# impromptuRong/hd_yolo

Measured on NVIDIA B200. Metric: postproc_tiles_per_s, higher is better.
Workload: dtype f32

## Files before the change

hd_yolo_b200/csrc/mask_regions.cu:

```cuda
#include "tma_common.cuh"
#include "mask_common.cuh"

namespace hdy {

constexpr int kRegBoxX = 24, kRegBoxY = 24;
constexpr int kRegNm = 32;
constexpr int kRegThreads = 256;
constexpr int kRegWarps = kRegThreads / 32;
constexpr int kRegList = 512;

template <typename E>
struct RegSmemT {
  E proto[kRegNm][kRegBoxY][kRegBoxX];
  float coef[kRegWarps][kRegNm];
  uint16_t list[kRegList];
  int nlist;
  int pad;
  uint64_t bar;
};
__device__ __forceinline__ float proto_f32(float v) { return v; }
__device__ __forceinline__ float proto_f32(__half v) { return __half2float(v); }

constexpr int kRegCap = 254;
constexpr int kMaxRegionsPerTile = 512;
struct RegionList {
  int32_t count;
  uint16_t det[kRegCap];
};
static_assert(sizeof(RegionList) == 512, "one region list is 512 bytes");
struct PmWorkspace {
  int32_t* large_count;
  int32_t* large_list;
  float* patches;
  RegionList* regions;
  int4* kr;
};
static inline size_t align256(size_t v) { return (v + 255) & ~(size_t)255; }
size_t process_mask_workspace_bytes(long long bs, long long max_det) {
  const long long slots = bs * max_det;
  return 256 + align256((size_t)slots * 4) + align256((size_t)slots * 16) +
         (size_t)slots * kPatchPitch * kPatchPitch * 4 + (size_t)bs * kMaxRegionsPerTile * sizeof(RegionList);
}
static PmWorkspace pm_workspace(void* base, long long slots) {
  PmWorkspace w;
  unsigned char* p = static_cast<unsigned char*>(base);
  w.large_count = reinterpret_cast<int32_t*>(p);
  p += 256;
  w.large_list = reinterpret_cast<int32_t*>(p);
  p += align256((size_t)slots * 4);
  w.kr = reinterpret_cast<int4*>(p);
  p += align256((size_t)slots * 16);
  w.patches = reinterpret_cast<float*>(p);
  p += (size_t)slots * kPatchPitch * kPatchPitch * 4;
  w.regions = reinterpret_cast<RegionList*>(p);
  return w;
}

struct KeptRange {
  float x1d, y1d, x2d, y2d;
  int px0, py0, px1, py1;
};
__device__ __forceinline__ KeptRange kept_range(const float4 b, float rx, float ry, int mw, int mh) {
  KeptRange k;
  k.x1d = __fmul_rn(b.x, rx);
  k.x2d = __fmul_rn(b.z, rx);
  k.y1d = __fmul_rn(b.y, ry);
  k.y2d = __fmul_rn(b.w, ry);
  k.px0 = ceil_to_int_clamped(k.x1d, 0, mw);
  k.px1 = ceil_to_int_clamped(k.x2d, 0, mw);
  k.py0 = ceil_to_int_clamped(k.y1d, 0, mh);
  k.py1 = ceil_to_int_clamped(k.y2d, 0, mh);
  if (!(k.x1d == k.x1d) || !(k.x2d == k.x2d) || !(k.y1d == k.y1d) || !(k.y2d == k.y2d)) k.px1 = k.px0, k.py1 = k.py0;
  return k;
}

__constant__ int c_inv16[17] = {0,     65536, 32768, 21846, 16384, 13108, 10923, 9363, 8192,
                                7282,  6554,  5958,  5462,  5042,  4682,  4370,  4096};

__global__ void __launch_bounds__(256) proto_bin_kernel(const float4* __restrict__ boxes,
                                                        const int32_t* __restrict__ counts, long long n_slots,
                                                        int max_det, int mh, int mw, int rxn, int ryn, float rx,
                                                        float ry, const int32_t* __restrict__ geom4,
                                                        RegionList* __restrict__ regions, int4* __restrict__ kr) {
  const long long slot = (long long)blockIdx.x * blockDim.x + threadIdx.x;
  if (slot >= n_slots) return;
  const int tile = (int)(slot / max_det), d = (int)(slot - (long long)tile * max_det);
  const bool live = d < counts[tile] && !(geom4 && (geom4[4 * slot + 2] <= 0 || geom4[4 * slot + 3] <= 0));
  KeptRange k;
  k.px0 = k.py0 = k.px1 = k.py1 = 0;
  if (live) k = kept_range(boxes[slot], rx, ry, mw, mh);
  kr[slot] = make_int4(k.px0, k.py0, k.px1, k.py1);
  if (k.px1 <= k.px0 || k.py1 <= k.py0) return;
  if (k.px1 - k.px0 > kPatchPitch || k.py1 - k.py0 > kPatchPitch) return;
  const int rx0 = k.px0 / kRegBoxX, rx1 = (k.px1 - 1) / kRegBoxX;
  const int ry0 = k.py0 / kRegBoxY, ry1 = (k.py1 - 1) / kRegBoxY;
  for (int ryy = ry0; ryy <= ry1; ++ryy)
    for (int rxx = rx0; rxx <= rx1; ++rxx) {
      RegionList& R = regions[(size_t)tile * (rxn * ryn) + ryy * rxn + rxx];
      const int pos = atomicAdd(&R.count, 1);
      if (pos < kRegCap) R.det[pos] = (uint16_t)d;
    }
}

template <typename E, typename Emit>
__device__ __forceinline__ void contract_piece(const E (*proto)[kRegBoxY][kRegBoxX], const float* __restrict__ coef_smem,
                                               const int4 kr, int X0, int Y0, int lane, Emit emit) {
  float cf[kRegNm];
#pragma unroll
  for (int c = 0; c < kRegNm; c += 4) {
    const float4 v = *reinterpret_cast<const float4*>(coef_smem + c);
    cf[c] = v.x;
    cf[c + 1] = v.y;
    cf[c + 2] = v.z;
    cf[c + 3] = v.w;
  }
  const int qx0 = max(kr.x, X0), qx1 = min(kr.z, X0 + kRegBoxX);
  const int qy0 = max(kr.y, Y0), qy1 = min(kr.w, Y0 + kRegBoxY);
  const int pw = qx1 - qx0;
  const int inv = c_inv16[pw];
  const int rows_per = (32 * inv) >> 16;
  const int ly = (lane * inv) >> 16, lx = lane - ly * pw;
  if (ly >= rows_per) return;
  const int xx = qx0 + lx, sx = xx - X0;
  for (int yy = qy0 + ly; yy < qy1; yy += rows_per) {
    const int sy = yy - Y0;
    float acc = 0.f;
#pragma unroll
    for (int c = 0; c < kRegNm; ++c) acc = fmaf(cf[c], proto_f32(proto[c][sy][sx]), acc);
    emit(xx - kr.x, yy - kr.y, sigmoidf_ref(acc));
  }
}

struct ListedRide {
  const void* protos;
  const float4* boxes;
  const int64_t* offsets;
  uint32_t* bits;
  int32_t* status;
  const int32_t* list;
  const int32_t* list_count;
  long long capacity_words;
  float rx, ry;
  int nm, mh, mw, ih, iw;
  int ctas;
};
constexpr int kListedTiles = 64;

template <typename E>
__global__ void __launch_bounds__(kRegThreads, 3) proto_patch_kernel(
    const __grid_constant__ CUtensorMap tmap, const float* __restrict__ coef, const int4* __restrict__ krs,
    const int32_t* __restrict__ counts, int max_det, int rxn, int ryn, float* __restrict__ patches,
    const RegionList* __restrict__ regions, const ListedRide LR) {
  extern __shared__ __align__(128) unsigned char smem_raw[];
  if ((int)blockIdx.x < LR.ctas) {
    float* stage = reinterpret_cast<float*>(smem_raw);
    process_mask_body<true, sizeof(E) == 2>(LR.protos, coef, LR.boxes, counts, max_det, LR.nm, LR.mh, LR.mw, LR.ih, LR.iw,
                                            1, LR.rx, LR.ry, nullptr, nullptr, LR.offsets, LR.bits, LR.capacity_words,
                                            LR.status, LR.list, (long long)*LR.list_count,
                                            (long long)(blockIdx.x / kListedTiles), (long long)(LR.ctas / kListedTiles),
                                            (int)(blockIdx.x % kListedTiles), kListedTiles, stage,
                                            stage + kPmStage * kPmStage);
    return;
  }
  const int bid = (int)blockIdx.x - LR.ctas;
  RegSmemT<E>& S = *reinterpret_cast<RegSmemT<E>*>(smem_raw);
  const int t = threadIdx.x, lane = t & 31, warp = t >> 5;
  const int per_tile = rxn * ryn;
  const int tile = bid / per_tile, reg = bid - tile * per_tile;
  const int RY = reg / rxn, RX = reg - RY * rxn;
  const int X0 = RX * kRegBoxX, Y0 = RY * kRegBoxY;
  const RegionList& RL = regions[bid];
  const int listed = RL.count;
  if (listed <= 0) return;
  const bool use_list = listed <= kRegCap;
  const int n = use_list ? listed : min(counts[tile], max_det);

  if (t == 0) {
    mbar_init(&S.bar, 1);
    asm volatile("fence.mbarrier_init.release.cluster;" ::: "memory");
    mbar_arrive_expect_tx(&S.bar, (uint32_t)sizeof(S.proto));
    tma_load_4d(&S.proto[0][0][0], &tmap, X0, Y0, 0, tile, &S.bar);
  }
  bool loaded = false;
  for (int base = 0; base < n; base += kRegList) {
    __syncthreads();
    if (t == 0) S.nlist = 0;
    __syncthreads();
    const int lim = min(base + kRegList, n);
    if (use_list) {
      for (int i = base + t; i < lim; i += kRegThreads) S.list[i - base] = RL.det[i];
      if (t == 0) S.nlist = lim - base;
    } else {
      for (int d = base + t; d < lim; d += kRegThreads) {
        const int4 k = krs[(size_t)tile * max_det + d];
        if (k.z <= k.x || k.w <= k.y) continue;
        if (k.z - k.x > kPatchPitch || k.w - k.y > kPatchPitch) continue;
        if (k.z <= X0 || k.x >= X0 + kRegBoxX || k.w <= Y0 || k.y >= Y0 + kRegBoxY) continue;
        S.list[atomicAdd(&S.nlist, 1)] = (uint16_t)(d - base);
      }
    }
    __syncthreads();
    const int nl = S.nlist;
    int e = warp;
    size_t nslot = 0;
    int4 nkr = make_int4(0, 0, 0, 0);
    float ncoef = 0.f;
    auto fetch = [&](int ee) {
      nslot = (size_t)tile * max_det + (use_list ? 0 : base) + S.list[ee];
      nkr = krs[nslot];
      ncoef = coef[nslot * kRegNm + lane];
    };
    if (e < nl) fetch(e);
    if (!loaded) {
      while (!mbar_try_wait(&S.bar, 0)) {
      }
      loaded = true;
    }
    for (; e < nl; e += kRegWarps) {
      const size_t slot = nslot;
      const int4 k = nkr;
      __syncwarp();
      S.coef[warp][lane] = ncoef;
      __syncwarp();
      if (e + kRegWarps < nl) fetch(e + kRegWarps);
      float* dst = patches + slot * (kPatchPitch * kPatchPitch);
      contract_piece<E>(S.proto, S.coef[warp], k, X0, Y0, lane,
                        [&](int px, int py, float v) { dst[py * kPatchPitch + px] = v; });
    }
  }
  if (!loaded) {
    while (!mbar_try_wait(&S.bar, 0)) {
    }
  }
}

constexpr int kUpWarps = 8;
constexpr int kPatchRing = kPatchPitch + 2;
constexpr int kRowChunk = 64;

struct RowTab {
  int i0, i1;
  float l0, l1;
};

struct UpSmem {
  float patch[kUpWarps][kPatchRing * kPatchRing];
  float col[kUpWarps][kPatchRing][32];
  RowTab rows[kUpWarps][kRowChunk];
};

template <bool PACKED, bool UPSAMPLE>
__global__ void __launch_bounds__(kUpWarps * 32) mask_upsample_pack_kernel(
    const float* __restrict__ patches, const float4* __restrict__ boxes, const int32_t* __restrict__ counts,
    long long n_slots, int max_det, int mh, int mw, int ih, int iw, float rx, float ry, float* __restrict__ out_dense,
    const int32_t* __restrict__ geom4, const int64_t* __restrict__ offsets, uint32_t* __restrict__ bits,
    long long capacity_words,
    int32_t* __restrict__ status, int32_t* __restrict__ large_count, int32_t* __restrict__ large_list) {
  static_assert(!(PACKED && UPSAMPLE), "the packed + upsampled form runs mask_upsample_pack2_kernel");
  __shared__ UpSmem S;
  const int lane = threadIdx.x & 31, warp = threadIdx.x >> 5;
  const long long slot = (long long)blockIdx.x * kUpWarps + warp;
  if (slot >= n_slots) return;
  const int tile = (int)(slot / max_det), d = (int)(slot - (long long)tile * max_det);
  if (d >= counts[tile]) return;
  PMGeom g;
  if (geom4) {
    const KeptRange k = kept_range(boxes[slot], rx, ry, mw, mh);
    const int4 wdw = reinterpret_cast<const int4*>(geom4)[slot];
    g.x1d = k.x1d, g.y1d = k.y1d, g.x2d = k.x2d, g.y2d = k.y2d;
    g.px0 = k.px0, g.py0 = k.py0, g.px1 = k.px1, g.py1 = k.py1;
    g.x0 = wdw.x, g.y0 = wdw.y, g.w = wdw.z, g.h = wdw.w;
  } else {
    g = pm_geometry(boxes[slot], mh, mw, ih, iw, UPSAMPLE ? 1 : 0, rx, ry);
  }
  if (g.w <= 0 || g.h <= 0) return;
  const int wpr = (g.w + 31) >> 5;
  const int oh = UPSAMPLE ? ih : mh, ow = UPSAMPLE ? iw : mw;
  long long off = 0;
  if (PACKED) {
    off = offsets[slot];
    if (off + (long long)wpr * g.h > capacity_words) {
      if (lane == 0) atomicOr(status, HDY_STATUS_OVERFLOW);
      return;
    }
  }
  const int pw = g.px1 - g.px0, ph = g.py1 - g.py0;
  if (pw > kPatchPitch || ph > kPatchPitch) {
    if (PACKED)
      for (long long i = lane; i < (long long)wpr * g.h; i += 32) bits[off + i] = 0u;
    if (lane == 0) large_list[atomicAdd(large_count, 1)] = (int32_t)slot;
    return;
  }
  float* P = S.patch[warp];
  {
    const float* src = patches + slot * (kPatchPitch * kPatchPitch);
#pragma unroll
    for (int i = lane; i < kPatchPitch * kPatchPitch; i += 32) {
      const int y = i >> 4, x = i & 15;
      P[(y + 1) * kPatchRing + x + 1] = (y < ph && x < pw) ? src[i] : 0.f;
    }
    for (int i = lane; i < 4 * kPatchRing; i += 32) {
      const int k = i / kPatchRing, j = i - k * kPatchRing;
      const int idx = k == 0 ? j : (k == 1 ? (kPatchRing - 1) * kPatchRing + j : (k == 2 ? j * kPatchRing : j * kPatchRing + kPatchRing - 1));
      P[idx] = 0.f;
    }
  }
  __syncwarp();

  if (!UPSAMPLE) {
    for (int w = 0; w < wpr; ++w) {
      const int c = (w << 5) + lane;
      const bool valid = c < g.w;
      for (int r = 0; r < g.h; ++r) {
        const bool bit = valid && P[(r + 1) * kPatchRing + (valid ? c + 1 : 0)] > 0.5f;
        if (PACKED) {
          const unsigned word = __ballot_sync(0xffffffffu, bit);
          if (lane == 0) bits[off + (long long)r * wpr + w] = word;
        } else if (valid) {
          out_dense[slot * oh * ow + (size_t)(g.y0 + r) * ow + g.x0 + c] = bit ? 1.f : 0.f;
        }
      }
    }
    return;
  }

  const float sxs = (float)mw / (float)iw, sys = (float)mh / (float)ih;
  RowTab* rowtab = S.rows[warp];
  float(*col)[32] = S.col[warp];
  const int src_rows = ph + 2;
  for (int r0 = 0; r0 < g.h; r0 += kRowChunk) {
    const int nr = min(kRowChunk, g.h - r0);
    __syncwarp();
    for (int r = lane; r < nr; r += 32) {
      const Lerp Y = lerp_coord(g.y0 + r0 + r, sys, mh);
      RowTab T;
      T.i0 = min(max(Y.i0 - g.py0 + 1, 0), ph + 1);
      T.i1 = min(max(Y.i1 - g.py0 + 1, 0), ph + 1);
      T.l0 = Y.l0;
      T.l1 = Y.l1;
      rowtab[r] = T;
    }
    __syncwarp();
    for (int w = 0; w < wpr; ++w) {
      const int vw = min(32, g.w - (w << 5));
      if (vw <= 16) {
        const int rows_per = 32 / vw;
        const int lr = lane / vw, lc = lane - lr * vw;
        const bool active = lr < rows_per;
        const Lerp X = lerp_coord(g.x0 + (w << 5) + lc, sxs, mw);
        const int xi0 = min(max(X.i0 - g.px0 + 1, 0), pw + 1), xi1 = min(max(X.i1 - g.px0 + 1, 0), pw + 1);
        __syncwarp();
        if (active)
          for (int s = lr; s < src_rows; s += rows_per)
            col[s][lc] = __fadd_rn(__fmul_rn(X.l0, P[s * kPatchRing + xi0]), __fmul_rn(X.l1, P[s * kPatchRing + xi1]));
        __syncwarp();
        for (int rb = 0; rb < nr; rb += rows_per) {
          const int r = rb + lr;
          if (active && r < nr) {
            const float4 rt = *reinterpret_cast<const float4*>(&rowtab[r]);
            const float v = __fadd_rn(__fmul_rn(rt.z, col[__float_as_int(rt.x)][lc]),
                                      __fmul_rn(rt.w, col[__float_as_int(rt.y)][lc]));
            out_dense[slot * oh * ow + (size_t)(g.y0 + r0 + r) * ow + g.x0 + (w << 5) + lc] = v > 0.5f ? 1.f : 0.f;
          }
        }
        continue;
      }
      const int c = (w << 5) + lane;
      const bool valid = c < g.w;
      const Lerp X = lerp_coord(g.x0 + (valid ? c : 0), sxs, mw);
      const int xi0 = min(max(X.i0 - g.px0 + 1, 0), pw + 1), xi1 = min(max(X.i1 - g.px0 + 1, 0), pw + 1);
      __syncwarp();
      for (int s = 0; s < src_rows; ++s)
        col[s][lane] = __fadd_rn(__fmul_rn(X.l0, P[s * kPatchRing + xi0]), __fmul_rn(X.l1, P[s * kPatchRing + xi1]));
      __syncwarp();
      float* dd = out_dense + slot * oh * ow + (size_t)(g.y0 + r0) * ow + g.x0 + c;
#pragma unroll 4
      for (int r = 0; r < nr; ++r) {
        const float4 rt = *reinterpret_cast<const float4*>(&rowtab[r]);
        const float v = __fadd_rn(__fmul_rn(rt.z, col[__float_as_int(rt.x)][lane]),
                                  __fmul_rn(rt.w, col[__float_as_int(rt.y)][lane]));
        if (valid) dd[(size_t)r * ow] = v > 0.5f ? 1.f : 0.f;
      }
    }
  }
}

constexpr int kV2Warps = 8;
constexpr int kV2Threads = kV2Warps * 32;
constexpr int kXRows = 20;
constexpr int kPairPitch = 2 * (kXRows + 1);
constexpr int kUpPitch = 24;
constexpr int kUpX0 = 4;

struct UpWarpSmem {
  float patch[kXRows * kUpPitch];
  float colT[16 * kPairPitch];
};

__device__ __forceinline__ unsigned long long f32x2_pack(float lo, float hi) {
  unsigned long long r;
  asm("mov.b64 %0, {%1, %2};" : "=l"(r) : "f"(lo), "f"(hi));
  return r;
}
__device__ __forceinline__ void f32x2_mul(unsigned long long a, unsigned long long b, float& lo, float& hi) {
  unsigned long long r;
  asm("mul.rn.f32x2 %0, %1, %2;" : "=l"(r) : "l"(a), "l"(b));
  asm("mov.b64 {%0, %1}, %2;" : "=f"(lo), "=f"(hi) : "l"(r));
}

__device__ __forceinline__ void up_zero_ring(float* P, int pw, int ph, int lane) {
  if (lane < kPatchRing) {
    P[kUpX0 - 1 + lane] = 0.f;
    P[(ph + 1) * kUpPitch + kUpX0 - 1 + lane] = 0.f;
    if (lane < ph) {
      P[(lane + 1) * kUpPitch + kUpX0 - 1] = 0.f;
      P[(lane + 1) * kUpPitch + kUpX0 + pw] = 0.f;
    }
  }
}

__device__ __forceinline__ void up_load_patch(float* P, const float* __restrict__ src, int pw, int ph, int lane) {
  const int row = lane >> 2, quad = lane & 3;
  const float4* s4 = reinterpret_cast<const float4*>(src);
  float4 a = make_float4(0.f, 0.f, 0.f, 0.f), b = a;
  const bool ra = row < ph, rb = row + 8 < ph;
  if (ra) a = s4[row * 4 + quad];
  if (rb) b = s4[(row + 8) * 4 + quad];
  if (ra) *reinterpret_cast<float4*>(P + (row + 1) * kUpPitch + kUpX0 + quad * 4) = a;
  if (rb) *reinterpret_cast<float4*>(P + (row + 9) * kUpPitch + kUpX0 + quad * 4) = b;
  __syncwarp();
  up_zero_ring(P, pw, ph, lane);
}

__device__ __forceinline__ void upsample_pack_v2(const float* __restrict__ P, float* __restrict__ colT, const int4 kr,
                                                 const int4 wdw, long long off, uint32_t* __restrict__ bits, int mh,
                                                 int mw, float sxs, float sys, int lane) {
  const int pw = kr.z - kr.x, ph = kr.w - kr.y;
  const int gx0 = wdw.x, gy0 = wdw.y, gw = wdw.z, gh = wdw.w;
  const int wpr = (gw + 31) >> 5;
  const int src_rows = ph + 2;
  for (int w = 0; w < wpr; ++w) {
    const int vw = min(32, gw - (w << 5));
    const int c = (w << 5) + lane;
    const Lerp X = lerp_coord(gx0 + (c < gw ? c : 0), sxs, mw);
    const float* p0 = P + kUpX0 - 1 + min(max(X.i0 - kr.x + 1, 0), pw + 1);
    const float* p1 = P + kUpX0 - 1 + min(max(X.i1 - kr.x + 1, 0), pw + 1);
    __syncwarp();
    float* ct = colT + (lane >> 1) * kPairPitch + (lane & 1);
    for (int s = 0; s < src_rows; s += 4) {
#pragma unroll
      for (int j = 0; j < 4; ++j)
        ct[(s + j) * 2] = __fadd_rn(__fmul_rn(X.l0, p0[(s + j) * kUpPitch]), __fmul_rn(X.l1, p1[(s + j) * kUpPitch]));
    }
    __syncwarp();
    for (int r0 = 0; r0 < gh; r0 += 32) {
      const int r = r0 + lane;
      const bool act = r < gh;
      const Lerp Y = lerp_coord(gy0 + (act ? r : 0), sys, mh);
      const float* c0 = colT + 2 * min(max(Y.i0 - kr.y + 1, 0), ph + 1);
      const float* c1 = colT + 2 * min(max(Y.i1 - kr.y + 1, 0), ph + 1);
      const unsigned long long W0 = f32x2_pack(Y.l0, Y.l0), W1 = f32x2_pack(Y.l1, Y.l1);
      uint32_t word = 0u;
#define HDY_SETBIT(v, x)                                                                                          \
  asm("{\n\t.reg .pred p;\n\tsetp.gt.f32 p, %1, 0f3F000000;\n\t@p or.b32 %0, %0, %2;\n\t}" : "+r"(word) : "f"(v), \
      "n"(1u << (x)));
#define HDY_PX2(x)                                                                                                \
  {                                                                                                               \
    float a0, a1, b0, b1;                                                                                         \
    f32x2_mul(W0, *reinterpret_cast<const unsigned long long*>(c0 + ((x) >> 1) * kPairPitch), a0, a1);            \
    f32x2_mul(W1, *reinterpret_cast<const unsigned long long*>(c1 + ((x) >> 1) * kPairPitch), b0, b1);            \
    const float v0 = __fadd_rn(a0, b0), v1 = __fadd_rn(a1, b1);                                                   \
    HDY_SETBIT(v0, (x))                                                                                           \
    HDY_SETBIT(v1, (x) + 1)                                                                                       \
  }
#define HDY_G4(g) HDY_PX2(g) HDY_PX2((g) + 2)
      HDY_G4(0)
      if (vw > 4) {
        HDY_G4(4)
        if (vw > 8) {
          HDY_G4(8)
          if (vw > 12) {
            HDY_G4(12)
            if (vw > 16) {
              HDY_G4(16)
              if (vw > 20) {
                HDY_G4(20)
                if (vw > 24) {
                  HDY_G4(24)
                  if (vw > 28) {
                    HDY_G4(28)
                  }
                }
              }
            }
          }
        }
      }
#undef HDY_G4
#undef HDY_PX2
#undef HDY_SETBIT
      if (vw < 32) word &= (1u << vw) - 1u;
      if (act) bits[off + (long long)r * wpr + w] = word;
    }
  }
}

__global__ void __launch_bounds__(256) proto_bin_fused_kernel(const float4* __restrict__ boxes,
                                                              const int32_t* __restrict__ counts, long long n_slots,
                                                              int max_det, int mh, int mw, int rxn, int ryn, float rx,
                                                              float ry, const int32_t* __restrict__ geom4,
                                                              RegionList* __restrict__ regions, int4* __restrict__ kr,
                                                              int32_t* __restrict__ large_count,
                                                              int32_t* __restrict__ large_list) {
  const long long slot = (long long)blockIdx.x * blockDim.x + threadIdx.x;
  if (slot >= n_slots) return;
  const int tile = (int)(slot / max_det), d = (int)(slot - (long long)tile * max_det);
  const bool live = d < counts[tile] && geom4[4 * slot + 2] > 0 && geom4[4 * slot + 3] > 0;
  KeptRange k;
  k.px0 = k.py0 = k.px1 = k.py1 = 0;
  if (live) k = kept_range(boxes[slot], rx, ry, mw, mh);
  bool leave = false;
  if (k.px1 > k.px0 && k.py1 > k.py0) {
    leave = k.px1 - k.px0 > kPatchPitch || k.py1 - k.py0 > kPatchPitch;
    if (!leave) {
      const int rx0 = k.px0 / kRegBoxX, rx1 = (k.px1 - 1) / kRegBoxX;
      const int ry0 = k.py0 / kRegBoxY, ry1 = (k.py1 - 1) / kRegBoxY;
      for (int ryy = ry0; ryy <= ry1; ++ryy)
        for (int rxx = rx0; rxx <= rx1; ++rxx) {
          RegionList& R = regions[(size_t)tile * (rxn * ryn) + ryy * rxn + rxx];
          const int pos = atomicAdd(&R.count, 1);
          if (pos < kRegCap)
            R.det[pos] = (uint16_t)d;
          else
            leave = true;
        }
    }
    if (leave) large_list[atomicAdd(large_count, 1)] = (int32_t)slot;
  }
  kr[slot] = leave ? make_int4(0, 0, 0, 0) : make_int4(k.px0, k.py0, k.px1, k.py1);
}

__global__ void pm_clear_listed_kernel(const int32_t* __restrict__ geom4, const int64_t* __restrict__ offsets,
                                       uint32_t* __restrict__ bits, long long capacity_words,
                                       const int32_t* __restrict__ list, const int32_t* __restrict__ list_count) {
  const int n = *list_count;
  for (int item = blockIdx.x; item < n; item += gridDim.x) {
    const long long slot = list[item];
    const int4 g = reinterpret_cast<const int4*>(geom4)[slot];
    const long long words = (long long)((g.z + 31) >> 5) * g.w, off = offsets[slot];
    if (off + words > capacity_words) continue;
    for (long long i = threadIdx.x; i < words; i += blockDim.x) bits[off + i] = 0u;
  }
}

__global__ void __launch_bounds__(kV2Threads) mask_upsample_pack2_kernel(
    const float* __restrict__ patches, const int4* __restrict__ krs, const int32_t* __restrict__ geom4,
    const int64_t* __restrict__ offsets, long long n_slots, int mh, int mw, float sxs, float sys,
    uint32_t* __restrict__ bits, long long capacity_words, int32_t* __restrict__ status) {
  __shared__ __align__(16) UpWarpSmem S[kV2Warps];
  const int lane = threadIdx.x & 31, warp = threadIdx.x >> 5;
  const long long slot = (long long)blockIdx.x * kV2Warps + warp;
  if (slot >= n_slots) return;
  const int4 kr = krs[slot];
  const int pw = kr.z - kr.x, ph = kr.w - kr.y;
  if (pw <= 0 || ph <= 0) return;
  const int4 wdw = reinterpret_cast<const int4*>(geom4)[slot];
  const long long off = offsets[slot];
  if (off + (long long)((wdw.z + 31) >> 5) * wdw.w > capacity_words) {
    if (lane == 0) atomicOr(status, HDY_STATUS_OVERFLOW);
    return;
  }
  float* P = S[warp].patch;
  up_load_patch(P, patches + slot * (kPatchPitch * kPatchPitch), pw, ph, lane);
  __syncwarp();
  upsample_pack_v2(P, S[warp].colT, kr, wdw, off, bits, mh, mw, sxs, sys, lane);
}

int launch_process_mask_regions(const void* protos, int proto_dtype, const float* coef, const float* boxes,
                                const int32_t* counts,
                                int bs, int max_det, int nm, int mh, int mw, int ih, int iw, int upsample, float rx,
                                float ry, float* out_dense, const int32_t* geom, const int64_t* offsets, uint32_t* bits,
                                long long capacity_words, int32_t* status, void* workspace, size_t workspace_bytes,
                                cudaStream_t stream) {
  const long long slots = (long long)bs * max_det;
  if (!workspace || workspace_bytes < process_mask_workspace_bytes(bs, max_det)) return 1;
  const bool half = proto_dtype == HDY_F16;
  const int esz = half ? 2 : 4;
  if (nm != kRegNm || (mw * esz & 15) != 0 || ((uintptr_t)protos & 15) != 0 || max_det > 65535) return 1;
  const bool packed = out_dense == nullptr;
  if (packed && upsample && !geom) return 1;
  const int rxn = (mw + kRegBoxX - 1) / kRegBoxX, ryn = (mh + kRegBoxY - 1) / kRegBoxY;
  if ((long long)bs * rxn * ryn >= (1ll << 31) || slots >= (1ll << 31) || rxn * ryn > kMaxRegionsPerTile) return 1;
  EncodeTiledFn enc = tensor_map_encoder();
  if (!enc) return 1;
  CUtensorMap map;
  const cuuint64_t dims[4] = {(cuuint64_t)mw, (cuuint64_t)mh, (cuuint64_t)nm, (cuuint64_t)bs};
  const cuuint64_t strides[3] = {(cuuint64_t)mw * esz, (cuuint64_t)mw * mh * esz, (cuuint64_t)mw * mh * nm * esz};
  const cuuint32_t box[4] = {kRegBoxX, kRegBoxY, kRegNm, 1};
  const cuuint32_t estr[4] = {1, 1, 1, 1};
  const CUresult r = enc(&map, half ? CU_TENSOR_MAP_DATA_TYPE_FLOAT16 : CU_TENSOR_MAP_DATA_TYPE_FLOAT32, 4,
                         const_cast<void*>(protos), dims, strides, box, estr,
                         CU_TENSOR_MAP_INTERLEAVE_NONE, CU_TENSOR_MAP_SWIZZLE_NONE, CU_TENSOR_MAP_L2_PROMOTION_L2_128B,
                         CU_TENSOR_MAP_FLOAT_OOB_FILL_NONE);
  if (r != CUDA_SUCCESS) return 1;
  const PmWorkspace W = pm_workspace(workspace, slots);
  cudaError_t e = cudaMemsetAsync(W.large_count, 0, 4, stream);
  if (e == cudaSuccess) e = cudaMemsetAsync(W.regions, 0, (size_t)bs * rxn * ryn * sizeof(RegionList), stream);
  if (e == cudaSuccess)
    e = half ? cudaFuncSetAttribute(proto_patch_kernel<__half>, cudaFuncAttributeMaxDynamicSharedMemorySize,
                                    (int)sizeof(RegSmemT<__half>))
             : cudaFuncSetAttribute(proto_patch_kernel<float>, cudaFuncAttributeMaxDynamicSharedMemorySize,
                                    (int)sizeof(RegSmemT<float>));
  if (e != cudaSuccess) {
    set_error("process_mask(regions) setup: %s", cudaGetErrorString(e));
    return HDY_ERR_CUDA;
  }
  const float4* b4 = reinterpret_cast<const float4*>(boxes);
  if (packed && upsample) {
    const float sxs = (float)mw / (float)iw, sys = (float)mh / (float)ih;
    proto_bin_fused_kernel<<<(unsigned)((slots + 255) / 256), 256, 0, stream>>>(
        b4, counts, slots, max_det, mh, mw, rxn, ryn, rx, ry, geom, W.regions, W.kr, W.large_count, W.large_list);
    pm_clear_listed_kernel<<<148, 256, 0, stream>>>(geom, offsets, bits, capacity_words, W.large_list, W.large_count);
    ListedRide LR;
    LR.protos = protos, LR.boxes = b4, LR.offsets = offsets, LR.bits = bits, LR.status = status;
    LR.list = W.large_list, LR.list_count = W.large_count, LR.capacity_words = capacity_words;
    LR.rx = rx, LR.ry = ry, LR.nm = nm, LR.mh = mh, LR.mw = mw, LR.ih = ih, LR.iw = iw;
    LR.ctas = kListedTiles * 9;
    const unsigned g1 = (unsigned)((long long)bs * rxn * ryn + LR.ctas);
    if (half)
      proto_patch_kernel<__half><<<g1, kRegThreads, sizeof(RegSmemT<__half>), stream>>>(
          map, coef, W.kr, counts, max_det, rxn, ryn, W.patches, W.regions, LR);
    else
      proto_patch_kernel<float><<<g1, kRegThreads, sizeof(RegSmemT<float>), stream>>>(
          map, coef, W.kr, counts, max_det, rxn, ryn, W.patches, W.regions, LR);
    mask_upsample_pack2_kernel<<<(unsigned)((slots + kV2Warps - 1) / kV2Warps), kV2Threads, 0, stream>>>(
        W.patches, W.kr, geom, offsets, slots, mh, mw, sxs, sys, bits, capacity_words, status);
    return check_launch("hdy_process_mask(packed)");
  }
  ListedRide no_ride;
  memset(&no_ride, 0, sizeof(no_ride));
  proto_bin_kernel<<<(unsigned)((slots + 255) / 256), 256, 0, stream>>>(b4, counts, slots, max_det, mh, mw, rxn, ryn, rx,
                                                                        ry, geom, W.regions, W.kr);
  if (half)
    proto_patch_kernel<__half><<<(unsigned)((long long)bs * rxn * ryn), kRegThreads, sizeof(RegSmemT<__half>), stream>>>(
        map, coef, W.kr, counts, max_det, rxn, ryn, W.patches, W.regions, no_ride);
  else
    proto_patch_kernel<float><<<(unsigned)((long long)bs * rxn * ryn), kRegThreads, sizeof(RegSmemT<float>), stream>>>(
        map, coef, W.kr, counts, max_det, rxn, ryn, W.patches, W.regions, no_ride);
  const unsigned g2 = (unsigned)((slots + kUpWarps - 1) / kUpWarps);
#define HDY_UP(P, U)                                                                                              \
  mask_upsample_pack_kernel<P, U><<<g2, kUpWarps * 32, 0, stream>>>(W.patches, b4, counts, slots, max_det, mh, mw, \
                                                                    ih, iw, rx, ry, out_dense, geom, offsets, bits, \
                                                                    capacity_words, status, W.large_count,         \
                                                                    W.large_list)
  if (packed)
    HDY_UP(true, false);
  else if (upsample)
    HDY_UP(false, true);
  else
    HDY_UP(false, false);
#undef HDY_UP
  int rc = check_launch("hdy_process_mask(regions)");
  if (rc) return rc;
  return launch_process_mask_listed(protos, proto_dtype, coef, boxes, counts, max_det, nm, mh, mw, ih, iw, upsample, rx, ry,
                                    out_dense, offsets, bits, capacity_words, status, W.large_list, W.large_count,
                                    stream);
}

}
```

Measured before the change: 152,600.

## Make packed upsample kernel persistent with atomic work-stealing over slot chunks

Turns mask_upsample_pack2_kernel into a persistent kernel sized to the occupancy limit. Each warp grabs chunks of slots from a global atomic ticket instead of owning one fixed slot. The goal is to spread uneven per-detection work (many empty or skipped slots) across warps and to avoid launching one warp per slot. In exchange it adds atomic contention, occupancy queries and a carveout attribute set on the host for each call, plus a launch-bounds hint that may limit registers.

```diff
diff --git a/hd_yolo_b200/csrc/mask_regions.cu b/hd_yolo_b200/csrc/mask_regions.cu
--- a/hd_yolo_b200/csrc/mask_regions.cu
+++ b/hd_yolo_b200/csrc/mask_regions.cu
@@ -1,3 +1,5 @@
+#include <algorithm>
+
 #include "tma_common.cuh"
 #include "mask_common.cuh"
 
@@ -30,6 +32,7 @@
 static_assert(sizeof(RegionList) == 512, "one region list is 512 bytes");
 struct PmWorkspace {
   int32_t* large_count;
+  uint32_t* ticket;
   int32_t* large_list;
   float* patches;
   RegionList* regions;
@@ -45,6 +48,7 @@
   PmWorkspace w;
   unsigned char* p = static_cast<unsigned char*>(base);
   w.large_count = reinterpret_cast<int32_t*>(p);
+  w.ticket = reinterpret_cast<uint32_t*>(p + 4);
   p += 256;
   w.large_list = reinterpret_cast<int32_t*>(p);
   p += align256((size_t)slots * 4);
@@ -553,27 +557,49 @@
   }
 }
 
-__global__ void __launch_bounds__(kV2Threads) mask_upsample_pack2_kernel(
+constexpr int kV2Chunk = 16;
+constexpr int kV2CtasPerSm = 6;
+__global__ void __launch_bounds__(kV2Threads, kV2CtasPerSm) mask_upsample_pack2_kernel(
     const float* __restrict__ patches, const int4* __restrict__ krs, const int32_t* __restrict__ geom4,
     const int64_t* __restrict__ offsets, long long n_slots, int mh, int mw, float sxs, float sys,
-    uint32_t* __restrict__ bits, long long capacity_words, int32_t* __restrict__ status) {
+    uint32_t* __restrict__ bits, long long capacity_words, int32_t* __restrict__ status,
+    uint32_t* __restrict__ ticket, int chunk) {
   __shared__ __align__(16) UpWarpSmem S[kV2Warps];
   const int lane = threadIdx.x & 31, warp = threadIdx.x >> 5;
-  const long long slot = (long long)blockIdx.x * kV2Warps + warp;
-  if (slot >= n_slots) return;
-  const int4 kr = krs[slot];
-  const int pw = kr.z - kr.x, ph = kr.w - kr.y;
-  if (pw <= 0 || ph <= 0) return;
-  const int4 wdw = reinterpret_cast<const int4*>(geom4)[slot];
-  const long long off = offsets[slot];
-  if (off + (long long)((wdw.z + 31) >> 5) * wdw.w > capacity_words) {
-    if (lane == 0) atomicOr(status, HDY_STATUS_OVERFLOW);
-    return;
-  }
   float* P = S[warp].patch;
-  up_load_patch(P, patches + slot * (kPatchPitch * kPatchPitch), pw, ph, lane);
-  __syncwarp();
-  upsample_pack_v2(P, S[warp].colT, kr, wdw, off, bits, mh, mw, sxs, sys, lane);
+  for (;;) {
+    uint32_t first = 0;
+    if (lane == 0) first = atomicAdd(ticket, (uint32_t)chunk);
+    first = __shfl_sync(0xffffffffu, first, 0);
+    if ((long long)first >= n_slots) return;
+    const long long last = min((long long)first + chunk, n_slots);
+    for (long long slot = first; slot < last; ++slot) {
+      const int4 kr = krs[slot];
+      const int pw = kr.z - kr.x, ph = kr.w - kr.y;
+      if (pw <= 0 || ph <= 0) continue;
+      const int4 wdw = reinterpret_cast<const int4*>(geom4)[slot];
+      const long long off = offsets[slot];
+      if (off + (long long)((wdw.z + 31) >> 5) * wdw.w > capacity_words) {
+        if (lane == 0) atomicOr(status, HDY_STATUS_OVERFLOW);
+        continue;
+      }
+      __syncwarp();
+      up_load_patch(P, patches + slot * (kPatchPitch * kPatchPitch), pw, ph, lane);
+      __syncwarp();
+      upsample_pack_v2(P, S[warp].colT, kr, wdw, off, bits, mh, mw, sxs, sys, lane);
+    }
+  }
+}
+
+static int upsample_pack2_grid() {
+  int dev = 0, sms = 0, per_sm = 0;
+  if (cudaGetDevice(&dev) != cudaSuccess ||
+      cudaDeviceGetAttribute(&sms, cudaDevAttrMultiProcessorCount, dev) != cudaSuccess ||
+      cudaFuncSetAttribute((const void*)mask_upsample_pack2_kernel, cudaFuncAttributePreferredSharedMemoryCarveout,
+                           cudaSharedmemCarveoutMaxShared) != cudaSuccess ||
+      cudaOccupancyMaxActiveBlocksPerMultiprocessor(&per_sm, mask_upsample_pack2_kernel, kV2Threads, 0) != cudaSuccess)
+    return 0;
+  return sms * per_sm;
 }
 
 int launch_process_mask_regions(const void* protos, int proto_dtype, const float* coef, const float* boxes,
@@ -604,7 +630,7 @@
                          CU_TENSOR_MAP_FLOAT_OOB_FILL_NONE);
   if (r != CUDA_SUCCESS) return 1;
   const PmWorkspace W = pm_workspace(workspace, slots);
-  cudaError_t e = cudaMemsetAsync(W.large_count, 0, 4, stream);
+  cudaError_t e = cudaMemsetAsync(W.large_count, 0, 8, stream);
   if (e == cudaSuccess) e = cudaMemsetAsync(W.regions, 0, (size_t)bs * rxn * ryn * sizeof(RegionList), stream);
   if (e == cudaSuccess)
     e = half ? cudaFuncSetAttribute(proto_patch_kernel<__half>, cudaFuncAttributeMaxDynamicSharedMemorySize,
@@ -633,8 +659,15 @@
     else
       proto_patch_kernel<float><<<g1, kRegThreads, sizeof(RegSmemT<float>), stream>>>(
           map, coef, W.kr, counts, max_det, rxn, ryn, W.patches, W.regions, LR);
-    mask_upsample_pack2_kernel<<<(unsigned)((slots + kV2Warps - 1) / kV2Warps), kV2Threads, 0, stream>>>(
-        W.patches, W.kr, geom, offsets, slots, mh, mw, sxs, sys, bits, capacity_words, status);
+    const int g2 = upsample_pack2_grid();
+    if (g2 <= 0) {
+      set_error("process_mask(packed): no occupancy for mask_upsample_pack2_kernel");
+      return HDY_ERR_CUDA;
+    }
+    const int chunk = (int)std::min<long long>(kV2Chunk, std::max<long long>(1, slots / (4ll * g2 * kV2Warps)));
+    mask_upsample_pack2_kernel<<<(unsigned)min((long long)g2, (slots + kV2Warps - 1) / kV2Warps), kV2Threads, 0,
+                                 stream>>>(W.patches, W.kr, geom, offsets, slots, mh, mw, sxs, sys, bits, capacity_words,
+                                           status, W.ticket, chunk);
     return check_launch("hdy_process_mask(packed)");
   }
   ListedRide no_ride;
```

Measured after the change: 161,200, median of 6. 5.6% higher.
